# pashtari/lrf

Measured on AMD Instinct MI355X. Metric: Mpixels/sec qmf_encode (8x8 patch, r=7, 10 iters), higher is better.
Workload: dtype f32; 1 GPU; 256 x 512x768x3 uint8 per GPU, YCbCr 4:2:0, 8x8 patches, ranks (7,3,3), bounds (-16,15), num_iters 10, int8 factors out (BASELINE configs[1]); priming_steps=3, global_batch=256, rank_input_bytes=301989888, parallelism=images sharded over 1 GPU(s), no data-path collective

## Files before the change

### lrf_amd/csrc/lrf_bcdp_kernel.hip

```cpp
#pragma once

#ifndef LRF_BCDP_MAX_POLLS
#define LRF_BCDP_MAX_POLLS (1 << 20)
#endif

struct BcdpSync {
    int head;
    int done;
    int err;
    int pad[29];
    int cell[1];
};

struct BcdpTabs {
    float *vf, *bf, *pp, *qp;
    const float* wf;
};

__device__ __forceinline__ float ld_sc1(const float* p) { return __hip_atomic_load((const LRF_GLOBAL float*)p, __ATOMIC_RELAXED, __HIP_MEMORY_SCOPE_AGENT); }
__device__ __forceinline__ void st_sc1(float* p, float v)
{
#ifdef LRF_BCDP_PLAIN_PSTORE
    *p = v;
#else
    __hip_atomic_store((LRF_GLOBAL float*)p, v, __ATOMIC_RELAXED, __HIP_MEMORY_SCOPE_AGENT);
#endif
}
typedef unsigned u32x4 __attribute__((ext_vector_type(4)));
typedef unsigned u32x2 __attribute__((ext_vector_type(2)));
__device__ __forceinline__ u32x4 ld_sc1_x4u(const void* base, unsigned off)
{
    const __amdgpu_buffer_rsrc_t rs = __builtin_amdgcn_make_buffer_rsrc(const_cast<void*>(base), (short)0, 0x7fffffff, 0x00020000);
    return __builtin_bit_cast(u32x4, __builtin_amdgcn_raw_buffer_load_b128(rs, off, 0, 16));
}
__device__ __forceinline__ f32x4 ld_sc1_x4(const float* base, unsigned off) { return __builtin_bit_cast(f32x4, ld_sc1_x4u(base, off)); }
__device__ __forceinline__ void st_sc1_x4(void* p, u32x4 v) { asm volatile("global_store_dwordx4 %0, %1, off sc1" ::"v"(p), "v"(v) : "memory"); }
__device__ __forceinline__ void st_sc1_x2(void* p, u32x2 v) { asm volatile("global_store_dwordx2 %0, %1, off sc1" ::"v"(p), "v"(v) : "memory"); }
__device__ __forceinline__ void st_sc1_b32(void* p, unsigned v) { asm volatile("global_store_dword %0, %1, off sc1" ::"v"(p), "v"(v) : "memory"); }
__device__ __forceinline__ void st_sc1_b16(void* p, unsigned v) { asm volatile("global_store_short %0, %1, off sc1" ::"v"(p), "v"(v) : "memory"); }
__device__ __forceinline__ void st_sc1_b8(void* p, unsigned v) { asm volatile("global_store_byte %0, %1, off sc1" ::"v"(p), "v"(v) : "memory"); }

__device__ __forceinline__ int bcdp_dense_chunks(int R) { return (64 * R + R * R + 3) >> 2; }
#define LRF_BCDP_USTAGE 544

__device__ __forceinline__ void bcdp_sum16(const PlaneDesc& pd, const float* __restrict__ Ppart, const float* __restrict__ Qpart, int lane,
                                           float (&acc)[16], float (&q)[4])
{
#pragma unroll
    for (int j = 0; j < 16; j++) acc[j] = 0.f;
#pragma unroll
    for (int j = 0; j < 4; j++) q[j] = 0.f;
    const float* Pp = Ppart + (long)pd.blk0 * 64 * LRF_RP + lane;
    const float* Qp = Qpart + (long)pd.blk0 * LRF_RP * LRF_RP + lane;
    constexpr int NB = 4;
    for (int b0 = 0; b0 < pd.nblk; b0 += NB) {
        float pv[NB][16], qv[NB][4];
#pragma unroll
        for (int k = 0; k < NB; k++) {
            const long blk = b0 + k < pd.nblk ? b0 + k : b0;
#pragma unroll
            for (int j = 0; j < 16; j++) pv[k][j] = ld_sc1(Pp + blk * 64 * LRF_RP + 64 * j);
#pragma unroll
            for (int j = 0; j < 4; j++) qv[k][j] = ld_sc1(Qp + blk * LRF_RP * LRF_RP + 64 * j);
        }
#pragma unroll
        for (int k = 0; k < NB; k++)
            if (b0 + k < pd.nblk) {
#pragma unroll
                for (int j = 0; j < 16; j++) acc[j] = (b0 + k == 0) ? pv[k][j] : acc[j] + pv[k][j];
#pragma unroll
                for (int j = 0; j < 4; j++) q[j] = (b0 + k == 0) ? qv[k][j] : q[j] + qv[k][j];
            }
    }
}
__device__ __forceinline__ void bcdp_wave_sync()
{
    __builtin_amdgcn_fence(__ATOMIC_RELEASE, "wavefront");
    __builtin_amdgcn_wave_barrier();
    __builtin_amdgcn_fence(__ATOMIC_ACQUIRE, "wavefront");
}

__device__ __forceinline__ void bcdp_sum_dense(const PlaneDesc& pd, const float* __restrict__ Ppart, int lane, float* sum_s)
{
    const int nch = bcdp_dense_chunks(pd.R), nj = (nch + 63) >> 6;
    const float* base = Ppart + (long)pd.blk0 * 64 * LRF_RP;
    f32x4 acc[3];
#pragma unroll
    for (int j = 0; j < 3; j++) acc[j] = (f32x4){0.f, 0.f, 0.f, 0.f};
    constexpr int NB = 4;
    for (int b0 = 0; b0 < pd.nblk; b0 += NB) {
        f32x4 pv[NB][3];
#pragma unroll
        for (int k = 0; k < NB; k++) {
            const unsigned blk = b0 + k < pd.nblk ? b0 + k : b0;
#pragma unroll
            for (int j = 0; j < 3; j++) {
                const int c = lane + 64 * j < nch ? lane + 64 * j : nch - 1;
                if (j < nj) pv[k][j] = ld_sc1_x4(base, (blk * 64 * LRF_RP + 4 * c) * 4);
            }
        }
#pragma unroll
        for (int k = 0; k < NB; k++)
            if (b0 + k < pd.nblk) {
#pragma unroll
                for (int j = 0; j < 3; j++)
                    if (j < nj) acc[j] = (b0 + k == 0) ? pv[k][j] : acc[j] + pv[k][j];
            }
    }
#pragma unroll
    for (int j = 0; j < 3; j++)
        if (lane + 64 * j < nch) *reinterpret_cast<f32x4*>(&sum_s[4 * (lane + 64 * j)]) = acc[j];
}

__device__ __forceinline__ void bcdp_vupdate(const PlaneDesc& pd, int pli, const float* __restrict__ Ppart, float* __restrict__ Vf,
                                             float* __restrict__ Bf, int8_t* __restrict__ V8, const GsParams gp, int write_i8, float* lds, int lane)
{
    float* a_s = lds;
    float* v_s = lds + 64 * LRF_RP;
    float* gt_s = lds + 2 * 64 * LRF_RP;
    float* sum_s = gt_s + LRF_GT_STRIDE;
    const int R = pd.R;
    bcdp_sum_dense(pd, Ppart, lane, sum_s);
    const float* Vg = Vf + (long)pli * 64 * LRF_RP;
#pragma unroll
    for (int j = 0; j < 4; j++) *reinterpret_cast<f32x4*>(&v_s[4 * (lane + 64 * j)]) = ld_sc1_x4(Vg, 16 * (lane + 64 * j));
    bcdp_wave_sync();
#pragma unroll
    for (int j = 0; j < 16; j++) {
        const int idx = lane + 64 * j, n = idx >> 4, r = idx & 15;
        a_s[idx] = r < R ? sum_s[r * 64 + n] : 0.f;
    }
#pragma unroll
    for (int j = 0; j < 4; j++) {
        const int idx = lane + 64 * j, jj = idx >> 4, r = idx & 15;
        if (jj < R && r < R) {
            const float q = sum_s[64 * R + jj * R + r];
            if (jj == r) {
                const float den = (q + 0.f) + LRF_EPS;
                gt_s[r * LRF_GT_LD + LRF_GT_DEN] = den;
                gt_s[r * LRF_GT_LD + LRF_GT_RDEN] = 1.0f / den;
            } else {
                gt_s[r * LRF_GT_LD + (jj < r ? jj : jj - 1)] = q;
            }
        }
    }
    __builtin_amdgcn_fence(__ATOMIC_RELEASE, "wavefront");
    __builtin_amdgcn_wave_barrier();
    __builtin_amdgcn_fence(__ATOMIC_ACQUIRE, "wavefront");
    {
        const bool native = (long)(R - 1) * 64 < 400;
        const float no_tab[17] = {0.f, 0.f, 0.f, 0.f, 0.f, 0.f, 0.f, 0.f, 0.f, 0.f, 0.f, 0.f, 0.f, 0.f, 0.f, 0.f, 0.f};
        gs_dispatch<8, false>(R, &a_s[lane * LRF_RP], &v_s[lane * LRF_RP], nullptr, 0, gt_s, native, gp, no_tab);
        float* Vp = Vf + (long)pli * 64 * LRF_RP + lane * LRF_RP;
        for (int r = 0; r < R; r++) st_sc1(Vp + r, v_s[lane * LRF_RP + r]);
        if (write_i8) {
            int8_t* vo = V8 + pd.v_off + (long)lane * R;
            for (int r = 0; r < R; r++) vo[r] = (int8_t)v_s[lane * LRF_RP + r];
        }
    }
    __builtin_amdgcn_fence(__ATOMIC_RELEASE, "wavefront");
    __builtin_amdgcn_wave_barrier();
    __builtin_amdgcn_fence(__ATOMIC_ACQUIRE, "wavefront");
    if (!write_i8) {
        float* gt_n = a_s;
        make_gtable(v_s, 64, R, gt_n, lane, 64);
        __builtin_amdgcn_fence(__ATOMIC_RELEASE, "wavefront");
        __builtin_amdgcn_wave_barrier();
        __builtin_amdgcn_fence(__ATOMIC_ACQUIRE, "wavefront");
        float* gt_g = Bf + (long)pli * LRF_GT_STRIDE;
        static_assert(LRF_GT_LD % 4 == 0, "the b table goes out in 16-B chunks");
        for (int i = 4 * lane; i < R * LRF_GT_LD; i += 256) st_sc1_x4(gt_g + i, *reinterpret_cast<const u32x4*>(&gt_n[i]));
    }
}


__device__ __forceinline__ void bcdp_vupdate16(const PlaneDesc& pd, int pli, const float* __restrict__ Ppart, const float* __restrict__ Qpart,
                                               float* __restrict__ Vf, float* __restrict__ Bf, int8_t* __restrict__ V8, const GsParams gp,
                                               int write_i8, float* lds, int lane)
{
    float* a_s = lds;
    float* v_s = lds + 64 * LRF_RP;
    float* gt_b = lds + 2 * 64 * LRF_RP;
    const int R = pd.R;
    {
        float acc[16], q[4];
        bcdp_sum16(pd, Ppart, Qpart, lane, acc, q);
#pragma unroll
        for (int j = 0; j < 16; j++) {
            a_s[lane + 64 * j] = acc[j];
            v_s[lane + 64 * j] = ld_sc1(Vf + (long)pli * 64 * LRF_RP + lane + 64 * j);
        }
#pragma unroll
        for (int j = 0; j < 4; j++) {
            const int idx = lane + 64 * j, jj = idx >> 4, r = idx & 15;
            if (jj < R && r < R) {
                if (jj == r) gt_b[r * LRF_GTB_LD + LRF_GTB_DEN] = (q[j] + 0.f) + LRF_EPS;
                else gt_b[r * LRF_GTB_LD + (jj < r ? jj : jj - 1)] = q[j];
            }
        }
    }
    bcdp_wave_sync();
    {
        float a[32], v[32];
#pragma unroll
        for (int j = 0; j < 16; j += 4) {
            const f32x4 va4 = *reinterpret_cast<const f32x4*>(&a_s[lane * LRF_RP + j]);
            const f32x4 vv4 = *reinterpret_cast<const f32x4*>(&v_s[lane * LRF_RP + j]);
#pragma unroll
            for (int i = 0; i < 4; i++) { a[j + i] = va4[i]; v[j + i] = vv4[i]; }
        }
#pragma unroll
        for (int j = 16; j < 32; j++) a[j] = v[j] = 0.f;
        mid_ordered_row(R, a, v, gt_b, gp.lo, gp.hi, std::make_integer_sequence<int, 16>{});
        float* Vp = Vf + (long)pli * 64 * LRF_RP + lane * LRF_RP;
        int8_t* vo = V8 + pd.v_off + (long)lane * R;
#pragma unroll
        for (int r = 0; r < 16; r++)
            if (r < R) {
                v_s[lane * LRF_RP + r] = v[r];
                st_sc1(Vp + r, v[r]);
                if (write_i8) vo[r] = (int8_t)v[r];
            }
    }
    bcdp_wave_sync();
    if (!write_i8) {
        float* gt_n = a_s;
        make_gtable(v_s, 64, R, gt_n, lane, 64);
        bcdp_wave_sync();
        float* gt_g = Bf + (long)pli * LRF_GT_STRIDE;
        for (int i = lane; i < R * LRF_GT_LD; i += 64) st_sc1(gt_g + i, gt_n[i]);
    }
}

__device__ __forceinline__ void bcdp_vupdate32(const PlaneDesc& pd, int pli, const float* __restrict__ Ppart, const float* __restrict__ Qpart,
                                               float* __restrict__ Vf, float* __restrict__ Bf, int8_t* __restrict__ V8, const GsParams gp,
                                               int write_i8, float* lds, int lane)
{
    float* t_s = lds;
    float* gt_b = lds + 64 * 32;
    const int R = pd.R;
    float a[32], v[32];
    {
        float acc[32], q[16];
#pragma unroll
        for (int m = 0; m < 32; m++) acc[m] = 0.f;
#pragma unroll
        for (int m = 0; m < 16; m++) q[m] = 0.f;
        const float* P0 = Ppart + (long)pd.blk0 * 64 * LRF_RPB + (lane >> 5) * LRF_RPB + (lane & 31);
        const float* Q0 = Qpart + (long)pd.blk0 * LRF_RPB * LRF_RPB + (lane >> 5) * LRF_RPB + (lane & 31);
        constexpr int NB = 2;
        for (int b0 = 0; b0 < pd.nblk; b0 += NB) {
            float pv[NB][32], qv[NB][16];
#pragma unroll
            for (int k = 0; k < NB; k++) {
                const long blk = b0 + k < pd.nblk ? b0 + k : b0;
#pragma unroll
                for (int m = 0; m < 32; m++) pv[k][m] = ld_sc1(P0 + blk * 64 * LRF_RPB + 2 * m * LRF_RPB);
#pragma unroll
                for (int m = 0; m < 16; m++) qv[k][m] = ld_sc1(Q0 + blk * LRF_RPB * LRF_RPB + 2 * m * LRF_RPB);
            }
#pragma unroll
            for (int k = 0; k < NB; k++)
                if (b0 + k < pd.nblk) {
#pragma unroll
                    for (int m = 0; m < 32; m++) acc[m] = (b0 + k == 0) ? pv[k][m] : acc[m] + pv[k][m];
#pragma unroll
                    for (int m = 0; m < 16; m++) q[m] = (b0 + k == 0) ? qv[k][m] : q[m] + qv[k][m];
                }
        }
#pragma unroll
        for (int m = 0; m < 32; m++) t_s[lane + 64 * m] = acc[m];
#pragma unroll
        for (int m = 0; m < 16; m++) {
            const int j = 2 * m + (lane >> 5), r = lane & 31;
            if (j < R && r < R) {
                if (j == r) gt_b[r * LRF_GTB_LD + LRF_GTB_DEN] = (q[m] + 0.f) + LRF_EPS;
                else gt_b[r * LRF_GTB_LD + (j < r ? j : j - 1)] = q[m];
            }
        }
    }
    bcdp_wave_sync();
#pragma unroll
    for (int j = 0; j < 32; j += 4) {
        const f32x4 t4 = *reinterpret_cast<const f32x4*>(&t_s[lane * 32 + j]);
#pragma unroll
        for (int i = 0; i < 4; i++) a[j + i] = t4[i];
    }
    bcdp_wave_sync();
    {
        const float* Vg = Vf + (long)pli * 64 * LRF_RPB + (lane >> 5) * LRF_RPB + (lane & 31);
        float vv[32];
#pragma unroll
        for (int m = 0; m < 32; m++) vv[m] = ld_sc1(Vg + 2 * m * LRF_RPB);
#pragma unroll
        for (int m = 0; m < 32; m++) t_s[lane + 64 * m] = vv[m];
    }
    bcdp_wave_sync();
#pragma unroll
    for (int j = 0; j < 32; j += 4) {
        const f32x4 t4 = *reinterpret_cast<const f32x4*>(&t_s[lane * 32 + j]);
#pragma unroll
        for (int i = 0; i < 4; i++) v[j + i] = t4[i];
    }
    mid_ordered_row(R, a, v, gt_b, gp.lo, gp.hi, std::make_integer_sequence<int, 32>{});
    bcdp_wave_sync();
    {
        int8_t* vo = V8 + pd.v_off + (long)lane * R;
#pragma unroll
        for (int r = 0; r < 32; r++) {
            t_s[lane * 32 + r] = r < R ? v[r] : 0.f;
            if (write_i8 && r < R) vo[r] = (int8_t)v[r];
        }
    }
    bcdp_wave_sync();
    {
        float* Vg = Vf + (long)pli * 64 * LRF_RPB + (lane >> 5) * LRF_RPB + (lane & 31);
        if ((lane & 31) < R) {
#pragma unroll
            for (int m = 0; m < 32; m++) st_sc1(Vg + 2 * m * LRF_RPB, t_s[lane + 64 * m]);
        }
    }
    if (!write_i8) {
        float* gt_g = Bf + (long)pli * LRF_GTB_STRIDE;
        for (int i = lane; i < R * R; i += 64) {
            const int j = i / R, r = i - j * R;
            float acc = 0.f;
#pragma unroll 8
            for (int k = 0; k < 64; k++) acc = fmaf(t_s[k * 32 + j], t_s[k * 32 + r], acc);
            if (j == r) st_sc1(gt_g + r * LRF_GTB_LD + LRF_GTB_DEN, (acc + 0.f) + LRF_EPS);
            else st_sc1(gt_g + r * LRF_GTB_LD + (j < r ? j : j - 1), acc);
        }
    }
}

template <int T>
__device__ __forceinline__ f32x4 mfma_quad(float a, float b, f32x4 acc) { return __builtin_amdgcn_mfma_f32_4x4x1f32(a, b, acc, 4, T, 0); }
template <int NC>
__device__ __forceinline__ void regs_times_quads(const f32x4 (&xv)[16], const float (&op)[4][4], f32x4 (&acc)[4])
{
    static_for<64>([&](auto kc) {
        constexpr int k = kc;
#pragma unroll
        for (int c = 0; c < NC; c++) acc[c] = mfma_quad<(k & 15)>(op[c][k >> 4], xv[k >> 2][k & 3], acc[c]);
    });
}
template <int NC>
__device__ __forceinline__ void row_times_quads(const float* xrow_lds, int g16, const float (&op)[4][4], f32x4 (&acc)[4])
{
    f32x4 xv[16];
    static_for<16>([&](auto Jc) {
        constexpr int J = Jc;
        xv[J] = *reinterpret_cast<const f32x4*>(reinterpret_cast<const char*>(xrow_lds) + ((16 * J) ^ g16));
    });
    __builtin_amdgcn_sched_barrier(0);
    regs_times_quads<NC>(xv, op, acc);
}
template <int Q>
__device__ __forceinline__ void xt_u_quads(const float* Xs, const float* us, int lane, f32x4 (&accP)[2])
{
    float uq[Q][4];
#pragma unroll
    for (int q = 0; q < Q; q++)
#pragma unroll
        for (int s = 0; s < 4; s++) uq[q][s] = us[(16 * s + (lane >> 2)) * 8 + 4 * q + (lane & 3)];
    const char* xb = reinterpret_cast<const char*>(Xs);
    const int l4 = 4 * lane;
    static_for<4>([&](auto sc) {
        constexpr int s = sc;
        float xc[16];
        static_for<16>([&](auto cc) {
            constexpr int c = cc;
            xc[c] = *reinterpret_cast<const float*>(xb + 256 * (16 * s + c) + (l4 ^ (16 * c)));
        });
        static_for<16>([&](auto cc) {
            constexpr int c = cc;
#pragma unroll
            for (int q = 0; q < Q; q++) accP[q] = mfma_quad<c>(uq[q][s], xc[c], accP[q]);
        });
    });
}

template <int MODE, bool BYTES>
__device__ __forceinline__ void bcdp_w_block(const float* __restrict__ X, const LumaSrc& ls, const PlaneDesc& pd, const BlockDesc& bd,
                                             const float* __restrict__ Vf, const float* __restrict__ Wf, const float* __restrict__ Bf,
                                             int8_t* __restrict__ U, float* __restrict__ Ppart, const GsParams& gp, float* Xs, const int lane)
{
    constexpr int RMAX = 8;
    const int li = lane & 15, lq = lane >> 4;
    float* us = Xs + 64 * 64;
    const float* uq = &us[(lq + 4 * (li >> 3)) * RMAX + (li & 7)];
    const float* xrow = &Xs[lane * 64];
    const int g16 = 16 * xsw(lane);
    const int R = pd.R;
    const float* Xp = X + pd.x_off + (long)bd.row0 * 64;
    const float* Vp = Vf + (long)bd.plane * 64 * LRF_RP;
    const float* gt = Bf + (long)bd.plane * LRF_GT_STRIDE;
    int8_t* Ub = U + pd.u_off + (long)bd.row0 * R;
    int nrows = pd.M - bd.row0;
    if (nrows > LRF_KC) nrows = LRF_KC;
    const int nsub = (nrows + 63) >> 6;
    const bool native = pd.native_t2_u != 0;

    const bool quads2 = R > 4;
    float vq[2][4], wq[2][4];
    {
        const int lr = lane & 3, lrow = lane >> 2;
#pragma unroll
        for (int q = 0; q < 2; q++)
#pragma unroll
            for (int s = 0; s < 4; s++) {
                vq[q][s] = 0.f;
                if (q == 0 || quads2) {
                    const f32x4 v4 = ld_sc1_x4(Vp, ((16 * s + lrow) * LRF_RP + 4 * q) * 4);
                    const float v = lr == 0 ? v4[0] : lr == 1 ? v4[1] : lr == 2 ? v4[2] : v4[3];
                    vq[q][s] = 4 * q + lr < R ? v : 0.f;
                }
                wq[q][s] = 0.f;
                if constexpr (MODE == 1) {
                    if (q == 0 || quads2) {
                        const float w = Wf[((long)bd.plane * 64 + 16 * s + lrow) * LRF_RP + 4 * q + lr];
                        wq[q][s] = 4 * q + lr < R ? w : 0.f;
                    }
                }
            }
    }
    static_assert(LRF_GT_LD % 4 == 0 && LRF_GT_RDEN % 4 == 0 && LRF_GT_DEN == LRF_GT_RDEN + 1, "b-table chunks");
    float tab[5];
    {
        const int tn = li & 7, e = tn < 7 ? (tn & 3) : 0;
        f32x4 t4[5];
#pragma unroll
        for (int j = 0; j < 4; j++) t4[j] = ld_sc1_x4(gt, ((2 * j + (li >> 3)) * LRF_GT_LD + (tn < 7 ? (tn & 4) : LRF_GT_RDEN)) * 4);
        t4[4] = ld_sc1_x4(gt, ((li & 7) * LRF_GT_LD + LRF_GT_RDEN) * 4);
#pragma unroll
        for (int j = 0; j < 4; j++) tab[j] = e == 0 ? t4[j][0] : e == 1 ? t4[j][1] : e == 2 ? t4[j][2] : t4[j][3];
        tab[4] = t4[4][1];
    }

    const bool x_nt = bd.x_nt != 0;
    f32x4 xq[4][4];
    auto issue_x_as = [&](auto ntc, int t, int T0, int T1, bool live) {
        constexpr bool NT = ntc;
        const int r0 = t * 64;
#pragma unroll
        for (int T = T0; T < T1; T++) {
#pragma unroll
            for (int q = 0; q < 4; q++) {
                int row = r0 + 16 * T + 4 * q + lq;
                row = row < nrows ? row : nrows - 1;
                const f32x4* src = reinterpret_cast<const f32x4*>(Xp + (long)row * 64 + 4 * li);
                if (live) xq[T][q] = NT ? __builtin_nontemporal_load(src) : *src;
                else xq[T][q] = (f32x4){0.f, 0.f, 0.f, 0.f};
            }
        }
    };
    auto issue_x = [&](int t, int T0, int T1, bool live) {
        if (x_nt) issue_x_as(std::true_type{}, t, T0, T1, live);
        else issue_x_as(std::false_type{}, t, T0, T1, live);
    };
    u32x2 by[3][8];
    __amdgpu_buffer_rsrc_t irs;
    if constexpr (BYTES)
        irs = __builtin_amdgcn_make_buffer_rsrc(const_cast<uint8_t*>(ls.img + (long)bd.plane * 3 * ls.hw), (short)0, 3 * ls.hw, 0x00020000);
    auto patch0_of = [&](int t) {
        int row = t * 64 + lane;
        row = row < nrows ? row : nrows - 1;
        return luma_patch_byte0(bd.row0 + row, ls.W, ls.nwl);
    };
    auto issue_b_as = [&](auto ntc, int p0, int j0, int j1) {
        constexpr int AUX = decltype(ntc)::value ? 2 : 0;
#pragma unroll
        for (int j = j0; j < j1; j++)
#pragma unroll
            for (int ch = 0; ch < 3; ch++)
                by[ch][j] = __builtin_bit_cast(u32x2, __builtin_amdgcn_raw_buffer_load_b64(irs, p0, ch * ls.hw + j * ls.W, AUX));
    };
    auto issue_b = [&](int p0, int j0, int j1) {
        if constexpr (BYTES) {
            if (x_nt) issue_b_as(std::true_type{}, p0, j0, j1);
            else issue_b_as(std::false_type{}, p0, j0, j1);
        }
    };
    uint8_t* ust = reinterpret_cast<uint8_t*>(Xs + 64 * 64 + 64 * RMAX);
    const uintptr_t uaddr = reinterpret_cast<uintptr_t>(Ub);
    const uint8_t* ub16 = reinterpret_cast<const uint8_t*>(uaddr & ~(uintptr_t)15);
    auto span_of = [&](int t, uintptr_t& a, int& len, int& nsl) {
        a = uaddr + (uintptr_t)(64 * R * t);
        const int nr = nrows - 64 * t;
        len = (nr < 64 ? nr : 64) * R;
        nsl = ((int)(a & 15) + len + 15) >> 4;
    };
    u32x4 uvec;
    int unsl = 0, uph = 0;
    auto issue_u = [&](int t) {
        uintptr_t a;
        int len;
        span_of(t, a, len, unsl);
        uph = (int)(a & 15);
        const int k = lane < unsl ? lane : unsl - 1;
        uvec = ld_sc1_x4u(ub16, (unsigned)((a & ~(uintptr_t)15) - reinterpret_cast<uintptr_t>(ub16)) + 16 * k);
    };
    auto row_bytes = [&](int ph, unsigned& lo, unsigned& hi) {
        const int o = ph + lane * R;
        const unsigned* w = reinterpret_cast<const unsigned*>(ust + (o & ~3));
        const unsigned w0 = w[0], w1 = w[1], w2 = w[2];
        lo = __builtin_amdgcn_alignbyte(w1, w0, (unsigned)(o & 3));
        hi = __builtin_amdgcn_alignbyte(w2, w1, (unsigned)(o & 3));
    };

    f32x4 accP[2], accQ = (f32x4){0.f, 0.f, 0.f, 0.f};
#pragma unroll
    for (int q = 0; q < 2; q++) accP[q] = (f32x4){0.f, 0.f, 0.f, 0.f};

#ifdef LRF_BCDP_PROBE_3Q
    const bool probe3q = bd.plane < (LRF_BCDP_PROBE_3Q);
#else
    constexpr bool probe3q = false;
#endif
    if constexpr (MODE == 0) issue_u(0);
    if constexpr (BYTES) {
        issue_b(patch0_of(0), 0, 8);
    } else {
        issue_x(0, 0, 3, true);
        if (!probe3q) issue_x(0, 3, 4, true);
    }
    for (int t = 0; t < nsub; t++) {
        const int r0 = t * 64;
        __builtin_amdgcn_sched_barrier(0);
        f32x4 xv[16];
        if constexpr (BYTES) {
#pragma unroll
            for (int J = 0; J < 16; J++) {
                const unsigned r = by[0][J >> 1][J & 1], g = by[1][J >> 1][J & 1], b = by[2][J >> 1][J & 1];
#pragma unroll
                for (int i = 0; i < 4; i++)
                    xv[J][i] = luma_of((float)((r >> (8 * i)) & 255u), (float)((g >> (8 * i)) & 255u), (float)((b >> (8 * i)) & 255u));
            }
#pragma unroll
            for (int J = 0; J < 16; J++)
                *reinterpret_cast<f32x4*>(reinterpret_cast<char*>(const_cast<float*>(xrow)) + ((16 * J) ^ g16)) = xv[J];
        } else {
#pragma unroll
            for (int T = 0; T < 4; T++)
#pragma unroll
                for (int q = 0; q < 4; q++) {
                    const int m = 16 * T + 4 * q + lq;
                    *reinterpret_cast<f32x4*>(&Xs[m * 64 + 4 * (li ^ (4 * q + lq))]) = xq[probe3q && T == 3 ? 2 : T][q];
                }
        }
        float u[RMAX];
        const int row = r0 + lane;
        int cph = 0;
        if constexpr (MODE == 0) {
            if (lane < unsl) *reinterpret_cast<u32x4*>(ust + 16 * lane) = uvec;
            cph = uph;
        }
        const int tn = t + 1;
        const bool more = tn < nsub;
        if constexpr (MODE == 0) {
            if (more) issue_u(tn);
        }
        int p0n = 0;
        if constexpr (BYTES) {
            if (more) {
                p0n = patch0_of(tn);
                issue_b(p0n, 0, 4);
            }
        } else
            issue_x(tn, 0, 2, more);
        __builtin_amdgcn_fence(__ATOMIC_RELEASE, "wavefront");
        __builtin_amdgcn_wave_barrier();
        __builtin_amdgcn_fence(__ATOMIC_ACQUIRE, "wavefront");
        if constexpr (MODE == 0) {
            unsigned lo, hi;
            row_bytes(cph, lo, hi);
#pragma unroll
            for (int r = 0; r < 4; r++) {
                u[r] = (float)(int)(int8_t)(lo >> (8 * r));
                u[4 + r] = (float)(int)(int8_t)(hi >> (8 * r));
            }
        }
        __builtin_amdgcn_sched_barrier(0);
        float a[RMAX];
        {
            f32x4 acc[4];
#pragma unroll
            for (int c = 0; c < 4; c++) acc[c] = (f32x4){0.f, 0.f, 0.f, 0.f};
            float op[4][4];
#pragma unroll
            for (int s = 0; s < 4; s++) {
                op[0][s] = vq[0][s];
                op[1][s] = vq[1][s];
                op[2][s] = wq[0][s];
                op[3][s] = wq[1][s];
            }
            auto rtq = [&](auto ncc) {
                constexpr int NC = ncc;
                if constexpr (BYTES) regs_times_quads<NC>(xv, op, acc);
                else row_times_quads<NC>(xrow, g16, op, acc);
            };
            if constexpr (MODE == 0) {
                if (quads2) rtq(std::integral_constant<int, 2>{});
                else rtq(std::integral_constant<int, 1>{});
            } else {
                if (quads2) rtq(std::integral_constant<int, 4>{});
                else {
#pragma unroll
                    for (int s = 0; s < 4; s++) op[1][s] = wq[0][s];
                    rtq(std::integral_constant<int, 2>{});
                    acc[2] = acc[1];
                    acc[1] = (f32x4){0.f, 0.f, 0.f, 0.f};
                }
            }
#pragma unroll
            for (int v = 0; v < 4; v++) {
                a[v] = acc[0][v];
                a[4 + v] = acc[1][v];
                if constexpr (MODE == 1) {
                    u[v] = acc[2][v];
                    u[4 + v] = acc[3][v];
                }
            }
        }
        if constexpr (BYTES) {
            if (more) issue_b(p0n, 4, 6);
        } else
            issue_x(tn, 2, 3, more);
        __builtin_amdgcn_sched_barrier(0);
        gs_regs_dispatch<RMAX>(R, a, u, tab, native, gp);
        if (row >= nrows) {
#pragma unroll
            for (int r = 0; r < RMAX; r++) u[r] = 0.f;
        }
        if constexpr (BYTES) {
            if (more) issue_b(p0n, 6, 8);
        } else if (!probe3q)
            issue_x(tn, 3, 4, more);
        __builtin_amdgcn_sched_barrier(0);
#pragma unroll
        for (int r = 0; r < RMAX; r += 4) *reinterpret_cast<f32x4*>(&us[lane * RMAX + r]) = (f32x4){u[r], u[r + 1], u[r + 2], u[r + 3]};
        uintptr_t sa;
        int slen, snsl;
        span_of(t, sa, slen, snsl);
        const int sph = (int)(sa & 15);
        if (row < nrows) {
            uint8_t* d = ust + sph + lane * R;
#pragma unroll
            for (int r = 0; r < RMAX; r++)
                if (r < R) d[r] = (uint8_t)(int)u[r];
        }
        __builtin_amdgcn_fence(__ATOMIC_RELEASE, "wavefront");
        __builtin_amdgcn_wave_barrier();
        __builtin_amdgcn_fence(__ATOMIC_ACQUIRE, "wavefront");
        if (lane < snsl) {
            const uintptr_t s0 = (sa & ~(uintptr_t)15) + 16 * lane;
            const uint8_t* src = ust + 16 * lane;
            int lo = lane == 0 ? sph : 0;
            const int hi = lane == snsl - 1 ? sph + slen - 16 * lane : 16;
            if (lo == 0 && hi == 16) {
                st_sc1_x4(reinterpret_cast<void*>(s0), *reinterpret_cast<const u32x4*>(src));
            } else {
                while (lo < hi) {
                    void* dst = reinterpret_cast<void*>(s0 + lo);
                    if ((lo & 7) == 0 && lo + 8 <= hi) {
                        st_sc1_x2(dst, *reinterpret_cast<const u32x2*>(src + lo));
                        lo += 8;
                    } else if ((lo & 3) == 0 && lo + 4 <= hi) {
                        st_sc1_b32(dst, *reinterpret_cast<const unsigned*>(src + lo));
                        lo += 4;
                    } else if ((lo & 1) == 0 && lo + 2 <= hi) {
                        st_sc1_b16(dst, *reinterpret_cast<const uint16_t*>(src + lo));
                        lo += 2;
                    } else {
                        st_sc1_b8(dst, src[lo]);
                        lo += 1;
                    }
                }
            }
        }
        __builtin_amdgcn_sched_barrier(0);
        float qu[8];
#pragma unroll
        for (int h = 0; h < 8; h++) qu[h] = uq[8 * h * RMAX];
#pragma unroll
        for (int h = 0; h < 8; h++) accQ = __builtin_amdgcn_mfma_f32_16x16x4f32(qu[h], qu[h], accQ, 0, 0, 0);
        if (quads2) xt_u_quads<2>(Xs, us, lane, accP);
        else xt_u_quads<1>(Xs, us, lane, accP);
        __builtin_amdgcn_sched_barrier(0);
        __builtin_amdgcn_fence(__ATOMIC_RELEASE, "wavefront");
        __builtin_amdgcn_wave_barrier();
        __builtin_amdgcn_fence(__ATOMIC_ACQUIRE, "wavefront");
    }
    float* ps = Xs;
#pragma unroll
    for (int q = 0; q < 2; q++)
#pragma unroll
        for (int v = 0; v < 4; v++)
            if (4 * q + v < R) ps[(4 * q + v) * 64 + lane] = accP[q][v];
#pragma unroll
    for (int reg = 0; reg < 4; reg++) {
        const int i = 4 * lq + reg;
        const float mine = accQ[reg];
        const float other = __shfl(mine, ((lq + 2) & 3) * 16 + ((li + 8) & 15), 64);
        if (i < R && li < R) ps[64 * R + i * R + li] = mine + other;
    }
    __builtin_amdgcn_fence(__ATOMIC_RELEASE, "wavefront");
    __builtin_amdgcn_wave_barrier();
    __builtin_amdgcn_fence(__ATOMIC_ACQUIRE, "wavefront");
    float* Pp = Ppart + ((long)pd.blk0 + bd.blk) * 64 * LRF_RP;
    const int nch = bcdp_dense_chunks(R);
    for (int c = lane; c < nch; c += 64) st_sc1_x4(Pp + 4 * c, *reinterpret_cast<const u32x4*>(&ps[4 * c]));
}

template <bool F16, int NP32, bool FIRST = false>
__global__ __launch_bounds__(64 * LRF_BCDW_WAVES) __attribute__((amdgpu_waves_per_eu(2, 2))) void k_bcd_p(
    const float* __restrict__ X, const PlaneDesc* __restrict__ planes, const BlockDesc* __restrict__ blocks, const BcdpTabs t16,
    const BcdpTabs t64, int8_t* __restrict__ U, int8_t* __restrict__ V8, GsParams gp, int nblocks, int niter, int nplanes, int plane0,
    BcdpSync* sync, int* err_host, int ncells, int seq, int wave_lds, const LumaSrc ls)
{
    extern __shared__ __attribute__((aligned(16))) float bcdp_lds[];
    const int wave = __builtin_amdgcn_readfirstlane(threadIdx.x >> 6);
    const int lane = threadIdx.x & 63;
    float* Xs = reinterpret_cast<float*>(reinterpret_cast<char*>(bcdp_lds) + wave * wave_lds);
    int* ticket = sync->cell;
    int* flag = sync->cell + nplanes;
    const int total = niter * nblocks;
    auto leave = [&]() {
        asm volatile("s_waitcnt vmcnt(0)" ::: "memory");
        int l = 0;
        if (lane == 0) l = __hip_atomic_fetch_add(&sync->done, 1, __ATOMIC_RELAXED, __HIP_MEMORY_SCOPE_AGENT);
        const int d = __builtin_amdgcn_readfirstlane(__shfl(l, 0, 64));
        if (d == (int)(gridDim.x * LRF_BCDW_WAVES) - 1) {
            for (int i = lane; i < ncells; i += 64) __hip_atomic_store(&sync->cell[i], 0, __ATOMIC_RELAXED, __HIP_MEMORY_SCOPE_AGENT);
            __hip_atomic_store(&sync->head, 0, __ATOMIC_RELAXED, __HIP_MEMORY_SCOPE_AGENT);
            __hip_atomic_store(&sync->done, 0, __ATOMIC_RELAXED, __HIP_MEMORY_SCOPE_AGENT);
        }
    };

    if (__hip_atomic_load(&sync->err, __ATOMIC_RELAXED, __HIP_MEMORY_SCOPE_AGENT) != 0) return;
    for (;;) {
        int idx_l = 0;
        if (lane == 0) idx_l = __hip_atomic_fetch_add(&sync->head, 1, __ATOMIC_RELAXED, __HIP_MEMORY_SCOPE_AGENT);
        const int idx = __builtin_amdgcn_readfirstlane(__shfl(idx_l, 0, 64));
        if (idx >= total) {
            leave();
            return;
        }
        const int it = idx / nblocks, blk = idx - it * nblocks;
#ifdef LRF_BCDP_DEBUG
        atomicAdd(&sync->cell[2 * nplanes + blk], 1 + 1000 * it);
#endif
        const BlockDesc bd = blocks[blk];
        const PlaneDesc pd = planes[bd.plane];
        const int pl = bd.plane - plane0;
        if (it > 0) {
            int polls = 0;
            while (__hip_atomic_load(&flag[pl], __ATOMIC_RELAXED, __HIP_MEMORY_SCOPE_AGENT) < it) {
                __builtin_amdgcn_s_sleep(8);
                if (++polls > LRF_BCDP_MAX_POLLS) {
                    __hip_atomic_store(&sync->err, 1, __ATOMIC_RELAXED, __HIP_MEMORY_SCOPE_AGENT);
                    __hip_atomic_store(err_host, seq, __ATOMIC_RELAXED, __HIP_MEMORY_SCOPE_SYSTEM);
                    return;
                }
            }
        }
        __atomic_signal_fence(__ATOMIC_SEQ_CST);
        asm volatile("" ::: "memory");
#ifdef LRF_BCDP_FENCES
        __builtin_amdgcn_fence(__ATOMIC_ACQUIRE, "agent");
        asm volatile("s_waitcnt vmcnt(0)" ::: "memory");
#endif
        int ln = lane;
        asm volatile("" : "+v"(ln));
        const int fam = (!F16 || pd.R <= 8) ? 0 : ((NP32 == 0 || pd.R <= 16) ? 1 : 2);
        static_assert(!FIRST || NP32 == 0, "the first iteration of ranks 17..32 stays a launch of its own (k_bcd_w32f)");
        const bool first = FIRST && it == 0;
        if (fam == 0) {
            constexpr bool kBytes = FIRST && !F16 && NP32 == 0;
            bool bytes = false;
            if constexpr (kBytes) bytes = bd.plane < ls.nluma;
            if (first) {
                if constexpr (FIRST) {
                    if constexpr (kBytes) {
                        if (bytes) bcdp_w_block<1, true>(X, ls, pd, bd, t16.vf, t16.wf, t16.bf, U, t16.pp, gp, Xs, ln);
                    }
                    if (!bytes) bcdp_w_block<1, false>(X, ls, pd, bd, t16.vf, t16.wf, t16.bf, U, t16.pp, gp, Xs, ln);
                }
            } else {
                if constexpr (kBytes) {
                    if (bytes) bcdp_w_block<0, true>(X, ls, pd, bd, t16.vf, nullptr, t16.bf, U, t16.pp, gp, Xs, ln);
                }
                if (!bytes) bcdp_w_block<0, false>(X, ls, pd, bd, t16.vf, nullptr, t16.bf, U, t16.pp, gp, Xs, ln);
            }
        }
        if constexpr (F16) {
            if (fam == 1) {
                if (first) {
                    if constexpr (FIRST) w16_block<1, MemSc1>(X, pd, bd, t16.vf, t16.wf, t16.bf, U, t16.pp, t16.qp, gp, Xs, ln);
                } else
                    w16_block<0, MemSc1>(X, pd, bd, t16.vf, nullptr, t16.bf, U, t16.pp, t16.qp, gp, Xs, ln);
            }
        }
        if constexpr (NP32 > 0) {
            if (fam == 2) w32_block<NP32, MemSc1>(X, pd, bd, t64.vf, t64.bf, U, t64.pp, t64.qp, gp, Xs, ln, 0);
        }
        asm volatile("s_waitcnt vmcnt(0)" ::: "memory");
#ifdef LRF_BCDP_FENCES
        __builtin_amdgcn_fence(__ATOMIC_RELEASE, "agent");
        asm volatile("s_waitcnt vmcnt(0)" ::: "memory");
#endif
        int arrived_l = 0;
        if (lane == 0) arrived_l = __hip_atomic_fetch_add(&ticket[pl], 1, __ATOMIC_RELAXED, __HIP_MEMORY_SCOPE_AGENT);
        const int arrived = __builtin_amdgcn_readfirstlane(__shfl(arrived_l, 0, 64));
        __atomic_signal_fence(__ATOMIC_SEQ_CST);
        asm volatile("" ::: "memory");
        if (arrived == (it + 1) * pd.nblk - 1) {
#ifdef LRF_BCDP_FENCES
            __builtin_amdgcn_fence(__ATOMIC_ACQUIRE, "agent");
            asm volatile("s_waitcnt vmcnt(0)" ::: "memory");
#endif
            const int last = it == niter - 1 ? 1 : 0;
            int lv = lane;
            asm volatile("" : "+v"(lv));
            if (fam == 0) bcdp_vupdate(pd, bd.plane, t16.pp, t16.vf, t16.bf, V8, gp, last, Xs, lv);
            if constexpr (F16) {
                if (fam == 1) bcdp_vupdate16(pd, bd.plane, t16.pp, t16.qp, t16.vf, t16.bf, V8, gp, last, Xs, lv);
            }
            if constexpr (NP32 > 0) {
                if (fam == 2) bcdp_vupdate32(pd, bd.plane, t64.pp, t64.qp, t64.vf, t64.bf, V8, gp, last, Xs, lv);
            }
            asm volatile("s_waitcnt vmcnt(0)" ::: "memory");
#ifdef LRF_BCDP_FENCES
            __builtin_amdgcn_fence(__ATOMIC_RELEASE, "agent");
            asm volatile("s_waitcnt vmcnt(0)" ::: "memory");
#endif
#ifdef LRF_BCDP_TEST_SKIP_FLAG
            if (!(pl == 0 && it == (FIRST ? 1 : 0) && niter == (FIRST ? 4 : 3)))
#endif
            __hip_atomic_store(&flag[pl], it + 1, __ATOMIC_RELAXED, __HIP_MEMORY_SCOPE_AGENT);
        }
    }
}
```

Measured before the change: 67480 Mpix/s.

## Defer byte-span stores and restructure the X/image prefetch pipeline with buffer loads

The per-tile loop is reorganised. Loads of X now go through a buffer resource whose out-of-bounds reads return zero, so the row clamping and the live/dead branching are gone and reads past the end are harmless. The global store of each tile's int8 factor span is deferred to the next iteration, after that iteration's loads are issued, so stores overlap the following tile's work. Staging of the current tile is split into two halves with the next tile's loads issued in between. The whole loop is also instantiated separately for the nontemporal and temporal cases, and the sc1 stores now use atomic builtins instead of inline asm. The aim is more overlap of memory latency with compute and fewer per-lane branches, at the cost of more code size and possible register pressure.

```diff
diff --git a/lrf_amd/csrc/lrf_bcdp_kernel.hip b/lrf_amd/csrc/lrf_bcdp_kernel.hip
--- a/lrf_amd/csrc/lrf_bcdp_kernel.hip
+++ b/lrf_amd/csrc/lrf_bcdp_kernel.hip
@@ -35,10 +35,12 @@
 }
 __device__ __forceinline__ f32x4 ld_sc1_x4(const float* base, unsigned off) { return __builtin_bit_cast(f32x4, ld_sc1_x4u(base, off)); }
 __device__ __forceinline__ void st_sc1_x4(void* p, u32x4 v) { asm volatile("global_store_dwordx4 %0, %1, off sc1" ::"v"(p), "v"(v) : "memory"); }
-__device__ __forceinline__ void st_sc1_x2(void* p, u32x2 v) { asm volatile("global_store_dwordx2 %0, %1, off sc1" ::"v"(p), "v"(v) : "memory"); }
-__device__ __forceinline__ void st_sc1_b32(void* p, unsigned v) { asm volatile("global_store_dword %0, %1, off sc1" ::"v"(p), "v"(v) : "memory"); }
-__device__ __forceinline__ void st_sc1_b16(void* p, unsigned v) { asm volatile("global_store_short %0, %1, off sc1" ::"v"(p), "v"(v) : "memory"); }
-__device__ __forceinline__ void st_sc1_b8(void* p, unsigned v) { asm volatile("global_store_byte %0, %1, off sc1" ::"v"(p), "v"(v) : "memory"); }
+__device__ __forceinline__ void st_sc1_x2(void* p, u32x2 v)
+{
+    __hip_atomic_store((LRF_GLOBAL unsigned long long*)p, __builtin_bit_cast(unsigned long long, v), __ATOMIC_RELAXED, __HIP_MEMORY_SCOPE_AGENT);
+}
+__device__ __forceinline__ void st_sc1_b16(void* p, unsigned v) { __hip_atomic_store((LRF_GLOBAL uint16_t*)p, (uint16_t)v, __ATOMIC_RELAXED, __HIP_MEMORY_SCOPE_AGENT); }
+__device__ __forceinline__ void st_sc1_b8(void* p, unsigned v) { __hip_atomic_store((LRF_GLOBAL uint8_t*)p, (uint8_t)v, __ATOMIC_RELAXED, __HIP_MEMORY_SCOPE_AGENT); }
 
 __device__ __forceinline__ int bcdp_dense_chunks(int R) { return (64 * R + R * R + 3) >> 2; }
 #define LRF_BCDP_USTAGE 544
@@ -437,26 +439,19 @@
         tab[4] = t4[4][1];
     }
 
-    const bool x_nt = bd.x_nt != 0;
+    const bool x_nt = __builtin_amdgcn_readfirstlane(bd.x_nt) != 0;
     f32x4 xq[4][4];
-    auto issue_x_as = [&](auto ntc, int t, int T0, int T1, bool live) {
-        constexpr bool NT = ntc;
-        const int r0 = t * 64;
+    const __amdgpu_buffer_rsrc_t xrs = __builtin_amdgcn_make_buffer_rsrc(const_cast<float*>(Xp), (short)0, nrows * 256, 0x00020000);
+    const unsigned xlane = (unsigned)(256 * lq + 16 * li);
+    auto issue_x = [&](auto ntc, int t, int T0, int T1) {
+        constexpr int AUX = decltype(ntc)::value ? 2 : 0;
+        const unsigned o = xlane + (unsigned)(t * 64 * 256);
 #pragma unroll
         for (int T = T0; T < T1; T++) {
 #pragma unroll
-            for (int q = 0; q < 4; q++) {
-                int row = r0 + 16 * T + 4 * q + lq;
-                row = row < nrows ? row : nrows - 1;
-                const f32x4* src = reinterpret_cast<const f32x4*>(Xp + (long)row * 64 + 4 * li);
-                if (live) xq[T][q] = NT ? __builtin_nontemporal_load(src) : *src;
-                else xq[T][q] = (f32x4){0.f, 0.f, 0.f, 0.f};
-            }
-        }
-    };
-    auto issue_x = [&](int t, int T0, int T1, bool live) {
-        if (x_nt) issue_x_as(std::true_type{}, t, T0, T1, live);
-        else issue_x_as(std::false_type{}, t, T0, T1, live);
+            for (int q = 0; q < 4; q++)
+                xq[T][q] = __builtin_bit_cast(f32x4, __builtin_amdgcn_raw_buffer_load_b128(xrs, o + (unsigned)((16 * T + 4 * q) * 256), 0, AUX));
+        }
     };
     u32x2 by[3][8];
     __amdgpu_buffer_rsrc_t irs;
@@ -465,21 +460,16 @@
     auto patch0_of = [&](int t) {
         int row = t * 64 + lane;
         row = row < nrows ? row : nrows - 1;
-        return luma_patch_byte0(bd.row0 + row, ls.W, ls.nwl);
+        const int p0 = luma_patch_byte0(bd.row0 + row, ls.W, ls.nwl);
+        return t < nsub ? p0 : 3 * ls.hw;
     };
-    auto issue_b_as = [&](auto ntc, int p0, int j0, int j1) {
+    auto issue_b = [&](auto ntc, int p0, int j0, int j1) {
         constexpr int AUX = decltype(ntc)::value ? 2 : 0;
 #pragma unroll
         for (int j = j0; j < j1; j++)
 #pragma unroll
             for (int ch = 0; ch < 3; ch++)
                 by[ch][j] = __builtin_bit_cast(u32x2, __builtin_amdgcn_raw_buffer_load_b64(irs, p0, ch * ls.hw + j * ls.W, AUX));
-    };
-    auto issue_b = [&](int p0, int j0, int j1) {
-        if constexpr (BYTES) {
-            if (x_nt) issue_b_as(std::true_type{}, p0, j0, j1);
-            else issue_b_as(std::false_type{}, p0, j0, j1);
-        }
     };
     uint8_t* ust = reinterpret_cast<uint8_t*>(Xs + 64 * 64 + 64 * RMAX);
     const uintptr_t uaddr = reinterpret_cast<uintptr_t>(Ub);
@@ -492,7 +482,8 @@
     };
     u32x4 uvec;
     int unsl = 0, uph = 0;
-    auto issue_u = [&](int t) {
+    auto issue_u = [&](int tq) {
+        const int t = tq < nsub ? tq : nsub - 1;
         uintptr_t a;
         int len;
         span_of(t, a, len, unsl);
@@ -507,151 +498,11 @@
         lo = __builtin_amdgcn_alignbyte(w1, w0, (unsigned)(o & 3));
         hi = __builtin_amdgcn_alignbyte(w2, w1, (unsigned)(o & 3));
     };
-
-    f32x4 accP[2], accQ = (f32x4){0.f, 0.f, 0.f, 0.f};
-#pragma unroll
-    for (int q = 0; q < 2; q++) accP[q] = (f32x4){0.f, 0.f, 0.f, 0.f};
-
-#ifdef LRF_BCDP_PROBE_3Q
-    const bool probe3q = bd.plane < (LRF_BCDP_PROBE_3Q);
-#else
-    constexpr bool probe3q = false;
-#endif
-    if constexpr (MODE == 0) issue_u(0);
-    if constexpr (BYTES) {
-        issue_b(patch0_of(0), 0, 8);
-    } else {
-        issue_x(0, 0, 3, true);
-        if (!probe3q) issue_x(0, 3, 4, true);
-    }
-    for (int t = 0; t < nsub; t++) {
-        const int r0 = t * 64;
-        __builtin_amdgcn_sched_barrier(0);
-        f32x4 xv[16];
-        if constexpr (BYTES) {
-#pragma unroll
-            for (int J = 0; J < 16; J++) {
-                const unsigned r = by[0][J >> 1][J & 1], g = by[1][J >> 1][J & 1], b = by[2][J >> 1][J & 1];
-#pragma unroll
-                for (int i = 0; i < 4; i++)
-                    xv[J][i] = luma_of((float)((r >> (8 * i)) & 255u), (float)((g >> (8 * i)) & 255u), (float)((b >> (8 * i)) & 255u));
-            }
-#pragma unroll
-            for (int J = 0; J < 16; J++)
-                *reinterpret_cast<f32x4*>(reinterpret_cast<char*>(const_cast<float*>(xrow)) + ((16 * J) ^ g16)) = xv[J];
-        } else {
-#pragma unroll
-            for (int T = 0; T < 4; T++)
-#pragma unroll
-                for (int q = 0; q < 4; q++) {
-                    const int m = 16 * T + 4 * q + lq;
-                    *reinterpret_cast<f32x4*>(&Xs[m * 64 + 4 * (li ^ (4 * q + lq))]) = xq[probe3q && T == 3 ? 2 : T][q];
-                }
-        }
-        float u[RMAX];
-        const int row = r0 + lane;
-        int cph = 0;
-        if constexpr (MODE == 0) {
-            if (lane < unsl) *reinterpret_cast<u32x4*>(ust + 16 * lane) = uvec;
-            cph = uph;
-        }
-        const int tn = t + 1;
-        const bool more = tn < nsub;
-        if constexpr (MODE == 0) {
-            if (more) issue_u(tn);
-        }
-        int p0n = 0;
-        if constexpr (BYTES) {
-            if (more) {
-                p0n = patch0_of(tn);
-                issue_b(p0n, 0, 4);
-            }
-        } else
-            issue_x(tn, 0, 2, more);
-        __builtin_amdgcn_fence(__ATOMIC_RELEASE, "wavefront");
-        __builtin_amdgcn_wave_barrier();
-        __builtin_amdgcn_fence(__ATOMIC_ACQUIRE, "wavefront");
-        if constexpr (MODE == 0) {
-            unsigned lo, hi;
-            row_bytes(cph, lo, hi);
-#pragma unroll
-            for (int r = 0; r < 4; r++) {
-                u[r] = (float)(int)(int8_t)(lo >> (8 * r));
-                u[4 + r] = (float)(int)(int8_t)(hi >> (8 * r));
-            }
-        }
-        __builtin_amdgcn_sched_barrier(0);
-        float a[RMAX];
-        {
-            f32x4 acc[4];
-#pragma unroll
-            for (int c = 0; c < 4; c++) acc[c] = (f32x4){0.f, 0.f, 0.f, 0.f};
-            float op[4][4];
-#pragma unroll
-            for (int s = 0; s < 4; s++) {
-                op[0][s] = vq[0][s];
-                op[1][s] = vq[1][s];
-                op[2][s] = wq[0][s];
-                op[3][s] = wq[1][s];
-            }
-            auto rtq = [&](auto ncc) {
-                constexpr int NC = ncc;
-                if constexpr (BYTES) regs_times_quads<NC>(xv, op, acc);
-                else row_times_quads<NC>(xrow, g16, op, acc);
-            };
-            if constexpr (MODE == 0) {
-                if (quads2) rtq(std::integral_constant<int, 2>{});
-                else rtq(std::integral_constant<int, 1>{});
-            } else {
-                if (quads2) rtq(std::integral_constant<int, 4>{});
-                else {
-#pragma unroll
-                    for (int s = 0; s < 4; s++) op[1][s] = wq[0][s];
-                    rtq(std::integral_constant<int, 2>{});
-                    acc[2] = acc[1];
-                    acc[1] = (f32x4){0.f, 0.f, 0.f, 0.f};
-                }
-            }
-#pragma unroll
-            for (int v = 0; v < 4; v++) {
-                a[v] = acc[0][v];
-                a[4 + v] = acc[1][v];
-                if constexpr (MODE == 1) {
-                    u[v] = acc[2][v];
-                    u[4 + v] = acc[3][v];
-                }
-            }
-        }
-        if constexpr (BYTES) {
-            if (more) issue_b(p0n, 4, 6);
-        } else
-            issue_x(tn, 2, 3, more);
-        __builtin_amdgcn_sched_barrier(0);
-        gs_regs_dispatch<RMAX>(R, a, u, tab, native, gp);
-        if (row >= nrows) {
-#pragma unroll
-            for (int r = 0; r < RMAX; r++) u[r] = 0.f;
-        }
-        if constexpr (BYTES) {
-            if (more) issue_b(p0n, 6, 8);
-        } else if (!probe3q)
-            issue_x(tn, 3, 4, more);
-        __builtin_amdgcn_sched_barrier(0);
-#pragma unroll
-        for (int r = 0; r < RMAX; r += 4) *reinterpret_cast<f32x4*>(&us[lane * RMAX + r]) = (f32x4){u[r], u[r + 1], u[r + 2], u[r + 3]};
+    auto store_span = [&](int t) {
         uintptr_t sa;
         int slen, snsl;
         span_of(t, sa, slen, snsl);
         const int sph = (int)(sa & 15);
-        if (row < nrows) {
-            uint8_t* d = ust + sph + lane * R;
-#pragma unroll
-            for (int r = 0; r < RMAX; r++)
-                if (r < R) d[r] = (uint8_t)(int)u[r];
-        }
-        __builtin_amdgcn_fence(__ATOMIC_RELEASE, "wavefront");
-        __builtin_amdgcn_wave_barrier();
-        __builtin_amdgcn_fence(__ATOMIC_ACQUIRE, "wavefront");
         if (lane < snsl) {
             const uintptr_t s0 = (sa & ~(uintptr_t)15) + 16 * lane;
             const uint8_t* src = ust + 16 * lane;
@@ -665,9 +516,6 @@
                     if ((lo & 7) == 0 && lo + 8 <= hi) {
                         st_sc1_x2(dst, *reinterpret_cast<const u32x2*>(src + lo));
                         lo += 8;
-                    } else if ((lo & 3) == 0 && lo + 4 <= hi) {
-                        st_sc1_b32(dst, *reinterpret_cast<const unsigned*>(src + lo));
-                        lo += 4;
                     } else if ((lo & 1) == 0 && lo + 2 <= hi) {
                         st_sc1_b16(dst, *reinterpret_cast<const uint16_t*>(src + lo));
                         lo += 2;
@@ -678,6 +526,159 @@
                 }
             }
         }
+    };
+
+    f32x4 accP[2], accQ = (f32x4){0.f, 0.f, 0.f, 0.f};
+#pragma unroll
+    for (int q = 0; q < 2; q++) accP[q] = (f32x4){0.f, 0.f, 0.f, 0.f};
+
+#ifdef LRF_BCDP_PROBE_3Q
+    const bool probe3q = bd.plane < (LRF_BCDP_PROBE_3Q);
+#else
+    constexpr bool probe3q = false;
+#endif
+    auto run = [&](auto ntc) {
+    __builtin_amdgcn_sched_barrier(0);
+    {
+        int p00 = 0;
+        if constexpr (BYTES) {
+            p00 = patch0_of(0);
+            issue_b(ntc, p00, 0, 4);
+        } else
+            issue_x(ntc, 0, 0, 2);
+        __builtin_amdgcn_sched_barrier(0);
+        if constexpr (MODE == 0) issue_u(0);
+        __builtin_amdgcn_sched_barrier(0);
+        if constexpr (BYTES) issue_b(ntc, p00, 4, 6);
+        else issue_x(ntc, 0, 2, 3);
+        __builtin_amdgcn_sched_barrier(0);
+        if constexpr (BYTES) issue_b(ntc, p00, 6, 8);
+        else if (!probe3q) issue_x(ntc, 0, 3, 4);
+    }
+    for (int t = 0; t < nsub; t++) {
+        const int r0 = t * 64;
+        const int tn = t + 1;
+        __builtin_amdgcn_sched_barrier(0);
+        f32x4 xv[16];
+        auto consume = [&](auto hc) {
+            constexpr int H = hc;
+            if constexpr (BYTES) {
+#pragma unroll
+                for (int J = 8 * H; J < 8 * H + 8; J++) {
+                    const unsigned r = by[0][J >> 1][J & 1], g = by[1][J >> 1][J & 1], b = by[2][J >> 1][J & 1];
+#pragma unroll
+                    for (int i = 0; i < 4; i++)
+                        xv[J][i] = luma_of((float)((r >> (8 * i)) & 255u), (float)((g >> (8 * i)) & 255u), (float)((b >> (8 * i)) & 255u));
+                }
+#pragma unroll
+                for (int J = 8 * H; J < 8 * H + 8; J++)
+                    *reinterpret_cast<f32x4*>(reinterpret_cast<char*>(const_cast<float*>(xrow)) + ((16 * J) ^ g16)) = xv[J];
+            } else {
+#pragma unroll
+                for (int T = 2 * H; T < 2 * H + 2; T++)
+#pragma unroll
+                    for (int q = 0; q < 4; q++) {
+                        const int m = 16 * T + 4 * q + lq;
+                        *reinterpret_cast<f32x4*>(&Xs[m * 64 + 4 * (li ^ (4 * q + lq))]) = xq[probe3q && T == 3 ? 2 : T][q];
+                    }
+            }
+        };
+        consume(std::integral_constant<int, 0>{});
+        __builtin_amdgcn_sched_barrier(0);
+        int p0n = 0;
+        if constexpr (BYTES) {
+            p0n = patch0_of(tn);
+            issue_b(ntc, p0n, 0, 4);
+        } else
+            issue_x(ntc, tn, 0, 2);
+        __builtin_amdgcn_sched_barrier(0);
+        consume(std::integral_constant<int, 1>{});
+        __builtin_amdgcn_sched_barrier(0);
+        if (t > 0) store_span(t - 1);
+        float u[RMAX];
+        const int row = r0 + lane;
+        int cph = 0;
+        if constexpr (MODE == 0) {
+            if (lane < unsl) *reinterpret_cast<u32x4*>(ust + 16 * lane) = uvec;
+            cph = uph;
+            issue_u(tn);
+        }
+        __builtin_amdgcn_fence(__ATOMIC_RELEASE, "wavefront");
+        __builtin_amdgcn_wave_barrier();
+        __builtin_amdgcn_fence(__ATOMIC_ACQUIRE, "wavefront");
+        if constexpr (MODE == 0) {
+            unsigned lo, hi;
+            row_bytes(cph, lo, hi);
+#pragma unroll
+            for (int r = 0; r < 4; r++) {
+                u[r] = (float)(int)(int8_t)(lo >> (8 * r));
+                u[4 + r] = (float)(int)(int8_t)(hi >> (8 * r));
+            }
+        }
+        __builtin_amdgcn_sched_barrier(0);
+        float a[RMAX];
+        {
+            f32x4 acc[4];
+#pragma unroll
+            for (int c = 0; c < 4; c++) acc[c] = (f32x4){0.f, 0.f, 0.f, 0.f};
+            float op[4][4];
+#pragma unroll
+            for (int s = 0; s < 4; s++) {
+                op[0][s] = vq[0][s];
+                op[1][s] = vq[1][s];
+                op[2][s] = wq[0][s];
+                op[3][s] = wq[1][s];
+            }
+            auto rtq = [&](auto ncc) {
+                constexpr int NC = ncc;
+                if constexpr (BYTES) regs_times_quads<NC>(xv, op, acc);
+                else row_times_quads<NC>(xrow, g16, op, acc);
+            };
+            if constexpr (MODE == 0) {
+                if (quads2) rtq(std::integral_constant<int, 2>{});
+                else rtq(std::integral_constant<int, 1>{});
+            } else {
+                if (quads2) rtq(std::integral_constant<int, 4>{});
+                else {
+#pragma unroll
+                    for (int s = 0; s < 4; s++) op[1][s] = wq[0][s];
+                    rtq(std::integral_constant<int, 2>{});
+                    acc[2] = acc[1];
+                    acc[1] = (f32x4){0.f, 0.f, 0.f, 0.f};
+                }
+            }
+#pragma unroll
+            for (int v = 0; v < 4; v++) {
+                a[v] = acc[0][v];
+                a[4 + v] = acc[1][v];
+                if constexpr (MODE == 1) {
+                    u[v] = acc[2][v];
+                    u[4 + v] = acc[3][v];
+                }
+            }
+        }
+        if constexpr (BYTES) issue_b(ntc, p0n, 4, 6);
+        else issue_x(ntc, tn, 2, 3);
+        __builtin_amdgcn_sched_barrier(0);
+        gs_regs_dispatch<RMAX>(R, a, u, tab, native, gp);
+        if (row >= nrows) {
+#pragma unroll
+            for (int r = 0; r < RMAX; r++) u[r] = 0.f;
+        }
+        if constexpr (BYTES) issue_b(ntc, p0n, 6, 8);
+        else if (!probe3q) issue_x(ntc, tn, 3, 4);
+        __builtin_amdgcn_sched_barrier(0);
+#pragma unroll
+        for (int r = 0; r < RMAX; r += 4) *reinterpret_cast<f32x4*>(&us[lane * RMAX + r]) = (f32x4){u[r], u[r + 1], u[r + 2], u[r + 3]};
+        if (row < nrows) {
+            uint8_t* d = ust + (int)((uaddr + (uintptr_t)(64 * R * t)) & 15) + lane * R;
+#pragma unroll
+            for (int r = 0; r < RMAX; r++)
+                if (r < R) d[r] = (uint8_t)(int)u[r];
+        }
+        __builtin_amdgcn_fence(__ATOMIC_RELEASE, "wavefront");
+        __builtin_amdgcn_wave_barrier();
+        __builtin_amdgcn_fence(__ATOMIC_ACQUIRE, "wavefront");
         __builtin_amdgcn_sched_barrier(0);
         float qu[8];
 #pragma unroll
@@ -691,6 +692,10 @@
         __builtin_amdgcn_wave_barrier();
         __builtin_amdgcn_fence(__ATOMIC_ACQUIRE, "wavefront");
     }
+    if (nsub > 0) store_span(nsub - 1);
+    };
+    if (x_nt) run(std::true_type{});
+    else run(std::false_type{});
     float* ps = Xs;
 #pragma unroll
     for (int q = 0; q < 2; q++)
```

Result: no change. 67090 Mpix/s (-0.6%).
